# claymore666/openhush

Measured on AMD Instinct MI355X. Metric: audio-sec/sec (xRT) large-v3 greedy, 30s chunks, 1/2/4/8 MI355X, higher is better.
Workload: dtype bf16; 1 GPU; large-v3 dims, steps of batch=32 x 30 s windows per GPU, greedy, 100 tokens/window (EOT suppressed), procedural weights seed 1234, every window a distinct synthetic recording, PCM resident in HBM; schedule LANES 4x3: 12 steps (384 windows) in flight per GPU - per lane ONE front-end pass and ONE decode batch of 96 rows, 4 decodes side by side on 64 CUs each; concurrent_sub_batches=1

## Files before the change

### include/ohw.h

```cpp
#ifndef OHW_H
#define OHW_H

#include <stddef.h>
#include <stdint.h>

#ifdef __cplusplus
extern "C" {
#endif

#define OHW_ABI_VERSION 2

enum {
  OHW_OK = 0,
  OHW_E_MODEL_NOT_FOUND = -3001,
  OHW_E_LOAD_FAILED = -3002,
  OHW_E_TRANSCRIBE = -3003,
  OHW_E_NO_GPU = -3004,
  OHW_E_OOM = -3005,
  OHW_E_INVALID_ARG = -3006,
  OHW_E_VALIDATION = -3007
};

enum { OHW_DTYPE_AUTO = -1, OHW_DTYPE_BF16 = 0, OHW_DTYPE_F16 = 1 };

// ... 464 lines not shown
int ohw_pool_set_fallback_device(ohw_pool* p, int on);
int ohw_pool_set_window_mode(ohw_pool* p, int mode);
int ohw_pool_set_initial_prompt(ohw_pool* p, const char* text);
int ohw_pool_set_hot_phrases(ohw_pool* p, const char* const* texts, const float* boosts, int n);
int ohw_pool_set_repetition(ohw_pool* p, float penalty, int ngram);
int ohw_pool_set_commands(ohw_pool* p, const char* const* texts, int n, float penalty);
int ohw_pool_set_best_of(ohw_pool* p, int n);
int ohw_pool_set_carry_context(ohw_pool* p, int max_tokens);
int ohw_pool_set_audio_ctx(ohw_pool* p, int n);
int ohw_pool_set_packed_encoder(ohw_pool* p, int on);
int ohw_pool_set_detect_language(ohw_pool* p, int on);
const char* ohw_pool_broadcast_note(const ohw_pool* p);
int ohw_pool_n_devices(const ohw_pool* p);
const char* ohw_pool_broadcast_kind(const ohw_pool* p);
ohw_engine* ohw_pool_engine(ohw_pool* p, int i);
void ohw_pool_free(ohw_pool* p);

const char* ohw_lang_id_to_code(int32_t id);
int32_t ohw_lang_code_to_id(const char* code);

const char* ohw_last_error(void);
int ohw_abi_version(void);
int ohw_state_fetch(ohw_state* st, const char* what, int batch, float* out, int64_t out_elems);
int ohw_ctx_weight_digest(const ohw_ctx* ctx, int index, char* name_out , uint64_t* digest);
int ohw_dequantize_host(int ttype, const void* blocks, int64_t n, float* out);
int ohw_dbg_dequantize(int device, int ttype, const void* blocks_host, int64_t n, float* out_host);
int ohw_dbg_gemm(int dtype, const void* A, const void* W, const float* bias, void* out, int64_t M, int64_t N,
                 int64_t K, int epilogue, void* stream);
int ohw_dbg_gemm_small(int dtype, const void* A, const void* W, const float* bias, void* out, int64_t M, int64_t N,
                       int64_t K, int epilogue, void* stream);
int ohw_dbg_attention(int dtype, const void* qkv, void* out, int batch, int T, int n_head, void* stream);
int ohw_dbg_attention_var(int dtype, const void* qkv, void* out, int batch, int T, int n_head, const int32_t* win_len_host,
                          const int32_t* win_off_host, void* stream);
enum { OHW_XA_PLAIN = 0, OHW_XA_SPLIT, OHW_XA_ROWS2, OHW_XA_ROWS3, OHW_XA_ROWS4, OHW_XA_GROUP2, OHW_XA_GROUP3, OHW_XA_GROUP4,
       OHW_XA_GROUP5, OHW_XA_GROUP_SPLIT };
enum { OHW_SA_PLAIN = 0, OHW_SA_SLOTS };
int ohw_dbg_cross_attn(int dtype, const void* q, const void* xk, const void* xv, void* out, int M, int n_new, int n_head, int t_len,
                       int kv_group, int batch_invariant, const int32_t* done_host, const int32_t* win_len_host, float* partials,
                       unsigned* tickets, int max_split_rows, int* variant_out, void* stream);
int ohw_dbg_cross_attn_chunk(int dtype, const void* q, const void* xk, const void* xv, void* out, int windows, int n_head, int t_len,
                             const int32_t* win_len_host, const int32_t* done_host, void* stream);
int ohw_dbg_cross_attn_chunk_n(int dtype, const void* q, const void* xk, const void* xv, void* out, int windows, int n_head, int t_len,
                               const int32_t* win_len_host, const int32_t* done_host, void* stream, int n_q);
int ohw_dbg_self_attn(int dtype, const void* q, const void* k_cache, const void* v_cache, const int32_t* n_past_host, void* out, int M,
                      int n_new, int n_head, int n_ctx, const int32_t* kv_slot_host, int* variant_out, void* stream);
int ohw_dbg_align_probs(int dtype, const void* q, const void* xk, int rows, int n_head, int t_len, int n_keys,
                        const int32_t* heads_host, int n_heads, float* p_out_host, void* stream);
int ohw_dbg_align_reduce(int device, const float* p_host, int n_heads, int n_all, int n_prompt, int n_keys, float* m_out_host);
int ohw_dbg_dtw(int device, const float* m_host, int n, int n_keys, int32_t* start_idx_out);
int ohw_dbg_poison(ohw_state* st, const char* what);
int ohw_dbg_vad_energy(ohw_state* st, const float* pcm, int64_t n, int pcm_on_device, float* e_out, int guard);
int ohw_dbg_vad_floor(ohw_state* st, const float* e, int64_t n_frames, const ohw_vad_detector* d, float* prob_out, int guard, float* floor_db_out);
int ohw_dbg_sample(ohw_state* st, const ohw_sample_params* p, const float* logits, const int32_t* history, int hist_stride,
                   const int32_t* n_hist, int batch, int32_t* tokens_out, float* logprobs_out, float* no_speech_out);
int ohw_dbg_sample_t(ohw_state* st, const ohw_sample_params* p, const float* logits, const int32_t* history, int hist_stride,
                     const int32_t* n_hist, int batch, float temperature, const double* uniforms, int32_t* tokens_out,
                     float* logprobs_out, float* no_speech_out);
int ohw_dbg_sample_group(ohw_state* st, const ohw_sample_params* p, const float* logits, const int32_t* history, int hist_stride,
                         const int32_t* n_hist, int n_windows, int group, int first, float temperature, const double* uniforms,
                         int32_t* done, int32_t* tokens_out, float* logprobs_out, float* no_speech_out, int32_t* win_done_out,
                         int32_t* n_cur_out);
int ohw_dbg_lang_pick(ohw_state* st, const float* logits, int batch, int32_t* ids_out, float* probs_out);
int ohw_dbg_counter(const ohw_state* st, const char* name);

#define OHW_DBG_SENTINEL_I32 (-7777777)
#define OHW_DBG_SENTINEL_F32 (-12345.0f)
// ... 133 lines not shown
```

### openhush_amd/csrc/attention.hip

```cpp
#include <type_traits>

#include "attention.hpp"

namespace ohw {

constexpr int ATT_THREADS = 256;
constexpr int ATT_QROWS = 128;
constexpr int ATT_KB = 64;

__device__ __forceinline__ int k_swz(int row) { return (row >> 1) & 7; }
__device__ __forceinline__ int v_swz(int row) { return ((row >> 1) & 1) << 2; }

enum AttMode { ATT_UNIFORM = 0, ATT_VAR = 1, ATT_PACKED = 2 };

template <typename T, int MODE>
__device__ __forceinline__ void encoder_attention_body(const T* __restrict__ qkv, T* __restrict__ out, int batch, int t_len, int n_head,
                                                       const int32_t* __restrict__ win_len, const int32_t* __restrict__ win_off) {
  using Ops = TypeOps<T>;
  using vec8 = typename Ops::vec8;
  __shared__ __attribute__((aligned(16))) unsigned char smem[2 * 16384];
  const int tid = threadIdx.x, lane = tid & 63, wave = tid >> 6;
  const int d = n_head * 64;
  const int64_t ld = 3 * (int64_t)d;
  const int nqb = (t_len + ATT_QROWS - 1) / ATT_QROWS;
  const unsigned nwg = (unsigned)(nqb * n_head * batch);
  const unsigned lid = xcd_remap(blockIdx.x, nwg);
  const int qb = lid % nqb;
  const int bh = lid / nqb;
  const int h = bh % n_head, b = bh / n_head;

  const int t_stride = t_len;
  int64_t row0 = (int64_t)b * t_stride;
  if (MODE == ATT_PACKED) {
    t_len = win_len[b];
    if (qb * ATT_QROWS >= t_len) return;
    row0 = win_off[b];
  }
  if (MODE == ATT_VAR) {
    t_len = win_len[b];
    if (qb * ATT_QROWS >= t_len) {
      const int r = qb * ATT_QROWS + (tid >> 1);
      if (r < t_stride) {
        u32x4* o = (u32x4*)(out + ((int64_t)b * t_stride + r) * d + h * 64 + (tid & 1) * 32);
        const u32x4 z = {0u, 0u, 0u, 0u};
#pragma unroll
        for (int i = 0; i < 4; ++i) o[i] = z;
      }
      return;
// ... 11 lines not shown

  const int skey = tid >> 3, schunk = tid & 7;
  const T* kg = base + d + h * 64 + schunk * 8;
  const T* vg = base + 2 * d + h * 64 + schunk * 8;
  int k_lds[2], v_lds[2];
#pragma unroll
  for (int i = 0; i < 2; ++i) {
    const int r = skey + 32 * i;
    k_lds[i] = r * 128 + ((schunk ^ k_swz(r)) << 4);
    v_lds[i] = 8192 + r * 128 + ((schunk ^ v_swz(r)) << 4);
  }
  const int nkb = (t_len + ATT_KB - 1) / ATT_KB;
  u32x4 rk[2][2], rv[2][2];
  auto gload = [&](auto set, int kb) {
    constexpr int S = decltype(set)::value;
#pragma unroll
    for (int i = 0; i < 2; ++i) {
      int key = kb * ATT_KB + skey + 32 * i;
      if (key > t_len - 1) key = t_len - 1;
      rk[S][i] = *(const u32x4*)(kg + (int64_t)key * ld);
      rv[S][i] = *(const u32x4*)(vg + (int64_t)key * ld);
    }
  };
  auto lstore = [&](auto set, int stage) {
    constexpr int S = decltype(set)::value;
#pragma unroll
    for (int i = 0; i < 2; ++i) {
      *(u32x4*)(smem + stage * 16384 + k_lds[i]) = rk[S][i];
      *(u32x4*)(smem + stage * 16384 + v_lds[i]) = rv[S][i];
    }
  };
  using Set0 = std::integral_constant<int, 0>;
  using Set1 = std::integral_constant<int, 1>;
  gload(Set0{}, 0);
  lstore(Set0{}, 0);
  __syncthreads();

  int k_rd[2];
#pragma unroll
  for (int kt = 0; kt < 2; ++kt) k_rd[kt] = (kt * 32 + ql) * 128;
  const int ksw = k_swz(ql);
  const int tq = (lane & 15) >> 2, tp = lane & 3, tg = (lane >> 4) & 1;

  f32x16 oacc[2];
#pragma unroll
  for (int i = 0; i < 2; ++i)
#pragma unroll
    for (int r = 0; r < 16; ++r) oacc[i][r] = 0.f;
  float m_run = -INFINITY, l_run = 0.f;
  const float sc = 0.125f * 1.44269504088896340736f;

  if (nkb > 1) gload(Set1{}, 1);
  auto block = [&](auto set, int kb) {
    constexpr int S = decltype(set)::value;
    const int cur = S * 16384;
    const bool more = kb + 1 < nkb;
    if (kb + 2 < nkb) gload(std::integral_constant<int, S>{}, kb + 2);

    f32x16 sacc[2];
#pragma unroll
    for (int kt = 0; kt < 2; ++kt) {
#pragma unroll
      for (int r = 0; r < 16; ++r) sacc[kt][r] = 0.f;
#pragma unroll
      for (int ks = 0; ks < 4; ++ks) {
        vec8 kf = *(const vec8*)(smem + cur + k_rd[kt] + (((2 * ks + hh) ^ ksw) << 4));
        sacc[kt] = Ops::mfma32(kf, qf[ks], sacc[kt]);
      }
    }
    const int key0 = kb * ATT_KB;
    if (key0 + ATT_KB > t_len) {
#pragma unroll
      for (int kt = 0; kt < 2; ++kt)
#pragma unroll
        for (int r = 0; r < 16; ++r) {
          const int key = key0 + kt * 32 + (r & 3) + 8 * (r >> 2) + 4 * hh;
          sacc[kt][r] = key < t_len ? sacc[kt][r] : -INFINITY;
        }
    }
    float bmax = -INFINITY;
#pragma unroll
    for (int kt = 0; kt < 2; ++kt)
#pragma unroll
      for (int r = 0; r < 16; ++r) bmax = fmaxf(bmax, sacc[kt][r]);
    bmax = fmaxf(bmax, __shfl_xor(bmax, 32, 64));
    const float m_new = fmaxf(m_run, bmax);
    if (!__all(m_new == m_run)) {
      const float alpha = __builtin_amdgcn_exp2f((m_run - m_new) * sc);
      l_run *= alpha;
#pragma unroll
// ... 4 lines not shown
    }
    const float m_sc = m_run * sc;
    float psum = 0.f;
#pragma unroll
    for (int kt = 0; kt < 2; ++kt)
#pragma unroll
      for (int r = 0; r < 16; ++r) {
        const float pv = __builtin_amdgcn_exp2f(__builtin_fmaf(sacc[kt][r], sc, -m_sc));
        sacc[kt][r] = pv;
        psum += pv;
      }
    l_run += psum;

#pragma unroll
    for (int sp = 0; sp < 4; ++sp) {
      const int kt = sp >> 1, s = sp & 1;
      union { vec8 v; unsigned u[4]; } pf;
#pragma unroll
      for (int j = 0; j < 4; ++j) pf.u[j] = pack2<T>(sacc[kt][8 * s + 2 * j], sacc[kt][8 * s + 2 * j + 1]);
      const int kbase = kt * 32 + 16 * s + 4 * hh + tq;
#pragma unroll
      for (int dt = 0; dt < 2; ++dt) {
        union { vec8 v; s16x4 h4[2]; } vf;
#pragma unroll
        for (int jj = 0; jj < 2; ++jj) {
          const int row = kbase + 8 * jj;
          const int colb = (dt * 32 + 16 * tg + 4 * tp) * 2;
          const int off = cur + 8192 + row * 128 + ((((colb >> 4) ^ v_swz(row)) << 4) | (colb & 15));
          vf.h4[jj] = __builtin_amdgcn_ds_read_tr16_b64_v4i16((__attribute__((address_space(3))) s16x4*)(smem + off));
        }
        oacc[dt] = Ops::mfma32(vf.v, pf.v, oacc[dt]);
      }
    }
    if (more) lstore(std::integral_constant<int, 1 - S>{}, 1 - S);
    __syncthreads();
  };
  for (int kb = 0; kb < nkb; kb += 2) {
    block(Set0{}, kb);
    if (kb + 1 < nkb) block(Set1{}, kb + 1);
  }

  l_run += __shfl_xor(l_run, 32, 64);
  const float inv = 1.0f / l_run;
  if (q_valid) {
    T* o = out + (row0 + q_row) * d + h * 64;
#pragma unroll
    for (int dt = 0; dt < 2; ++dt)
#pragma unroll
      for (int g = 0; g < 4; ++g) {
        u32x2 w;
        w.x = pack2<T>(oacc[dt][4 * g] * inv, oacc[dt][4 * g + 1] * inv);
        w.y = pack2<T>(oacc[dt][4 * g + 2] * inv, oacc[dt][4 * g + 3] * inv);
        *(u32x2*)(o + dt * 32 + 8 * g + 4 * hh) = w;
      }
  }
}

template <typename T, bool VAR>
__global__ __launch_bounds__(ATT_THREADS, 2) void encoder_attention_kernel(const T* __restrict__ qkv, T* __restrict__ out,
                                                                          int batch, int t_len, int n_head, const int32_t* __restrict__ win_len) {
  encoder_attention_body<T, VAR ? ATT_VAR : ATT_UNIFORM>(qkv, out, batch, t_len, n_head, win_len, nullptr);
}
template <typename T>
__global__ __launch_bounds__(ATT_THREADS, 2) void encoder_attention_packed_kernel(const T* __restrict__ qkv, T* __restrict__ out, int batch, int t_len, int n_head,
                                                                                 const int32_t* __restrict__ win_len, const int32_t* __restrict__ win_off) {
  encoder_attention_body<T, ATT_PACKED>(qkv, out, batch, t_len, n_head, win_len, win_off);
}

template <typename T>
void launch_encoder_attention(const void* qkv, void* out, int batch, int t_len, int n_head, hipStream_t stream, const int32_t* win_len, const int32_t* win_off) {
  const int nqb = (t_len + ATT_QROWS - 1) / ATT_QROWS;
  const unsigned nwg = (unsigned)(nqb * n_head * batch);
  if (win_off && !win_len) throw Error(OHW_E_INVALID_ARG, "attention: packed rows need the windows' lengths");
  if (win_off)
    hipLaunchKernelGGL((encoder_attention_packed_kernel<T>), dim3(nwg), dim3(ATT_THREADS), 0, stream, (const T*)qkv, (T*)out, batch, t_len, n_head, win_len, win_off);
  else if (win_len)
    hipLaunchKernelGGL((encoder_attention_kernel<T, true>), dim3(nwg), dim3(ATT_THREADS), 0, stream, (const T*)qkv, (T*)out, batch, t_len, n_head, win_len);
  else
    hipLaunchKernelGGL((encoder_attention_kernel<T, false>), dim3(nwg), dim3(ATT_THREADS), 0, stream, (const T*)qkv, (T*)out, batch, t_len, n_head, win_len);
  HIP_CHECK(hipGetLastError());
}
template void launch_encoder_attention<bf16_t>(const void*, void*, int, int, int, hipStream_t, const int32_t*, const int32_t*);
template void launch_encoder_attention<f16_t>(const void*, void*, int, int, int, hipStream_t, const int32_t*, const int32_t*);

}
```

### openhush_amd/csrc/attention.hpp

```cpp
#pragma once
#include "common.hpp"

namespace ohw {
template <typename T> void launch_encoder_attention(const void* qkv, void* out, int batch, int t_len, int n_head, hipStream_t stream,
                                                    const int32_t* win_len = nullptr, const int32_t* win_off = nullptr);
}
```

### openhush_amd/csrc/engine.hip

```cpp
#include <execinfo.h>
#include <signal.h>
#include <unistd.h>

#include <cstring>
#include <memory>
#include <mutex>
#include <shared_mutex>
#include <type_traits>
#include <vector>
#include <algorithm>

#include "attention.hpp"
#include "dequant.hpp"
#include "gemm.hpp"
#include "kernels.hpp"
#include "logit_rules.hpp"
#include "model.hpp"

namespace ohw {
ohw_ctx* ctx_from_file(const char* path, int device, int dtype);
ohw_ctx* ctx_synthetic(const ohw_hparams* hp, uint32_t seed, int device, int dtype);
ohw_ctx* ctx_shell(const ohw_hparams* hp, int device, int dtype);
void select_device(int device);

// ... 3152 lines not shown
    HIP_CHECK(hipStreamSynchronize(nullptr));
    HIP_CHECK(hipMemcpy(out_host, out.p, (size_t)n * 4, hipMemcpyDeviceToHost));
  });
}

int ohw_dbg_poison(ohw_state* st, const char* what) {
  return guard([&] {
    if (!st || !what) throw Error(OHW_E_INVALID_ARG, "null argument");
    const std::string w = what;
    const DevBuf* buf = w == "qkv" ? &st->qkv : w == "att" ? &st->att : nullptr;
    if (!buf) throw Error(OHW_E_INVALID_ARG, std::string("poison: unknown buffer '") + what + "'");
    HIP_CHECK(hipSetDevice(st->ctx->device));
    HIP_CHECK(hipMemsetAsync(buf->p, 0xff, buf->bytes, st->stream));
  });
}

int ohw_dbg_attention(int dtype, const void* qkv, void* out, int batch, int T, int n_head, void* stream) {
  return guard([&] {
    Dispatch::run(dtype, [&](auto* tag) {
      using TT = std::remove_pointer_t<decltype(tag)>;
      launch_encoder_attention<TT>(qkv, out, batch, T, n_head, (hipStream_t)stream);
    });
  });
}

static void dbg_upload(DevBuf& buf, const int32_t* host, size_t n) {
  buf.alloc(n * sizeof(int32_t));
  HIP_CHECK(hipMemcpy(buf.p, host, n * sizeof(int32_t), hipMemcpyHostToDevice));
}
static void dbg_check_dtype(int dtype, const char* what) {
  if (dtype != OHW_DTYPE_BF16 && dtype != OHW_DTYPE_F16) throw Error(OHW_E_INVALID_ARG, std::string(what) + ": dtype must be 0 (bf16) or 1 (f16)");
}

int ohw_dbg_attention_var(int dtype, const void* qkv, void* out, int batch, int T, int n_head, const int32_t* win_len_host,
                          const int32_t* win_off_host, void* stream) {
  return guard([&] {
    dbg_check_dtype(dtype, "dbg_attention_var");
    if (!qkv || !out || batch < 1 || T < 1 || n_head < 1) throw Error(OHW_E_INVALID_ARG, "dbg_attention_var: null buffer, or batch, T or n_head below 1");
    if (win_off_host && !win_len_host) throw Error(OHW_E_INVALID_ARG, "dbg_attention_var: packed rows (win_off) need the windows' lengths (win_len)");
    int64_t sum = 0;
    for (int b = 0; win_len_host && b < batch; ++b) {
      if (win_len_host[b] < 1 || win_len_host[b] > T)
        throw Error(OHW_E_INVALID_ARG, "dbg_attention_var: win_len[" + std::to_string(b) + "] = " + std::to_string(win_len_host[b]) + " is outside 1 .. T = " + std::to_string(T));
      if (win_off_host && win_off_host[b] != sum)
        throw Error(OHW_E_INVALID_ARG, "dbg_attention_var: win_off[" + std::to_string(b) + "] = " + std::to_string(win_off_host[b]) +
                                           " is not the exclusive prefix sum of win_len (" + std::to_string(sum) + ")");
      sum += win_len_host[b];
    }
    DevBuf len, off;
    if (win_len_host) dbg_upload(len, win_len_host, (size_t)batch);
    if (win_off_host) dbg_upload(off, win_off_host, (size_t)batch);
    Dispatch::run(dtype, [&](auto* tag) {
      using TT = std::remove_pointer_t<decltype(tag)>;
      launch_encoder_attention<TT>(qkv, out, batch, T, n_head, (hipStream_t)stream, win_len_host ? len.as<int32_t>() : nullptr,
                                   win_off_host ? off.as<int32_t>() : nullptr);
    });
    HIP_CHECK(hipStreamSynchronize((hipStream_t)stream));
  });
}

int ohw_dbg_cross_attn(int dtype, const void* q, const void* xk, const void* xv, void* out, int M, int n_new, int n_head, int t_len,
                       int kv_group, int batch_invariant, const int32_t* done_host, const int32_t* win_len_host, float* partials,
                       unsigned* tickets, int max_split_rows, int* variant_out, void* stream) {
  return guard([&] {
    dbg_check_dtype(dtype, "dbg_cross_attn");
    if (!q || !xk || !xv || !out || M < 1 || n_new < 1 || n_head < 1 || t_len < 1)
      throw Error(OHW_E_INVALID_ARG, "dbg_cross_attn: null buffer, or M, n_new, n_head or t_len below 1");
    if (kv_group < 1 || kv_group > 5) throw Error(OHW_E_INVALID_ARG, "dbg_cross_attn: kv_group must be 1 .. 5 (beams per window)");
    if (kv_group > 1 && n_new != 1) throw Error(OHW_E_INVALID_ARG, "dbg_cross_attn: beams (kv_group > 1) are single-token rows: n_new must be 1");
    if (M % n_new != 0) throw Error(OHW_E_INVALID_ARG, "dbg_cross_attn: M must be a multiple of n_new");
    if (kv_group > 1 && M % kv_group != 0) throw Error(OHW_E_INVALID_ARG, "dbg_cross_attn: M must be a multiple of kv_group");
    if ((partials == nullptr) != (tickets == nullptr)) throw Error(OHW_E_INVALID_ARG, "dbg_cross_attn: partials and tickets come together");
    if (partials && !batch_invariant && !win_len_host && (max_split_rows < 1 || M > max_split_rows))
      throw Error(OHW_E_INVALID_ARG, "dbg_cross_attn: M = " + std::to_string(M) + " rows exceed max_split_rows = " + std::to_string(max_split_rows) +
                                         ", the rows the partials and tickets hold");
    const int windows = kv_group > 1 ? M / kv_group : M / n_new;
    for (int w = 0; win_len_host && w < windows; ++w)
      if (win_len_host[w] < 1 || win_len_host[w] > t_len)
        throw Error(OHW_E_INVALID_ARG, "dbg_cross_attn: win_len[" + std::to_string(w) + "] = " + std::to_string(win_len_host[w]) + " is outside 1 .. t_len = " + std::to_string(t_len));
    DevBuf done, len;
    if (done_host) dbg_upload(done, done_host, (size_t)windows);
    if (win_len_host) dbg_upload(len, win_len_host, (size_t)windows);
    int variant = -1;
    Dispatch::run(dtype, [&](auto* tag) {
      using TT = std::remove_pointer_t<decltype(tag)>;
      variant = launch_cross_attn<TT>(q, xk, xv, out, M, n_new, n_head, t_len, partials, tickets, max_split_rows,
                                      done_host ? done.as<int32_t>() : nullptr, (hipStream_t)stream, kv_group, batch_invariant != 0,
                                      win_len_host ? len.as<int32_t>() : nullptr);
    });
    HIP_CHECK(hipStreamSynchronize((hipStream_t)stream));
// ... 337 lines not shown
```

### openhush_amd/engine.py

```python
from __future__ import annotations

import ctypes as C
import dataclasses
import os
import time
from typing import List, Optional, Sequence, Tuple, Union

import numpy as np

_HERE = os.path.dirname(os.path.abspath(__file__))
LIB_PATH = os.environ.get("OHW_LIB") or os.path.join(_HERE, "libohw.so")

CHUNK_SAMPLES = 480000
CHUNK_FRAMES = 3000

OHW_DTYPE_AUTO, OHW_DTYPE_BF16, OHW_DTYPE_F16 = -1, 0, 1
OHW_MEL_REFLECT, OHW_MEL_ZERO_TAIL = 0, 1
OHW_WINDOW_FIXED, OHW_WINDOW_SEEK, OHW_WINDOW_FIXED_RECORDING_MEL = 0, 1, 2
OHW_SCHEDULE_SEQUENTIAL, OHW_SCHEDULE_PIPELINE, OHW_SCHEDULE_LANES = 0, 1, 2
EPI_BIAS_T, EPI_BIAS_GELU_T, EPI_BIAS_RESID_F32, EPI_F32 = 0, 1, 2, 4
XA_PLAIN, XA_SPLIT, XA_ROWS2, XA_ROWS3, XA_ROWS4, XA_GROUP2, XA_GROUP3, XA_GROUP4, XA_GROUP5, XA_GROUP_SPLIT = range(10)
SA_PLAIN, SA_SLOTS = 0, 1

OHW_E_MODEL_NOT_FOUND, OHW_E_LOAD_FAILED, OHW_E_TRANSCRIBE = -3001, -3002, -3003
OHW_E_NO_GPU, OHW_E_OOM, OHW_E_INVALID_ARG, OHW_E_VALIDATION = -3004, -3005, -3006, -3007


class HParams(C.Structure):
    _fields_ = [(n, C.c_int32) for n in ("n_vocab", "n_audio_ctx", "n_audio_state", "n_audio_head", "n_audio_layer",
                                         "n_text_ctx", "n_text_state", "n_text_head", "n_text_layer", "n_mels", "ftype")]

    def as_list(self):
        return [int(getattr(self, n)) for n, _ in self._fields_]


class SpecialTokens(C.Structure):
    _fields_ = [(n, C.c_int32) for n in ("eot", "sot", "translate", "transcribe", "solm", "prev", "nosp", "no_timestamps",
                                         "timestamp_begin", "blank", "n_langs")]


class AudioInfo(C.Structure):
    _fields_ = [("error", C.c_int32), ("duration_secs", C.c_float), ("sample_count", C.c_int64), ("min_value", C.c_float),
                ("max_value", C.c_float), ("rms", C.c_float), ("nan_count", C.c_int64), ("inf_count", C.c_int64)]


class SampleParams(C.Structure):
    _fields_ = [(n, C.c_int32) for n in ("lang_id", "translate", "no_timestamps", "suppress_blank", "max_initial_ts", "n_max", "force_len")]


class PreprocessConfig(C.Structure):
    _fields_ = [("preprocessing", C.c_int32), ("normalization_enabled", C.c_int32), ("normalization_target_db", C.c_float),
                ("compression_enabled", C.c_int32), ("compression_threshold_db", C.c_float), ("compression_ratio", C.c_float),
                ("compression_attack_ms", C.c_float), ("compression_release_ms", C.c_float), ("compression_makeup_gain_db", C.c_float),
                ("limiter_enabled", C.c_int32), ("limiter_ceiling_db", C.c_float), ("limiter_release_ms", C.c_float)]

# ... 431 lines not shown


AUDIO_ERRORS = {0: "Ok", 1: "Empty", 2: "InvalidSampleRate", 3: "TooLong", 4: "TooShort", 5: "ContainsNaN", 6: "ContainsInfinite"}

EXPORTS = [
    "ohw_validate_audio", "ohw_ctx_create", "ohw_ctx_create_synthetic", "ohw_ctx_info", "ohw_token_text", "ohw_ctx_free",
    "ohw_state_create", "ohw_state_free", "ohw_state_set_stream", "ohw_state_max_batch", "ohw_mel", "ohw_recording_set", "ohw_mel_seek", "ohw_encode", "ohw_decode",
    "ohw_default_sample_params", "ohw_sample_greedy_host", "ohw_greedy", "ohw_state_timings", "ohw_engine_new",
    "ohw_engine_transcribe", "ohw_engine_last_tokens", "ohw_engine_benchmark", "ohw_engine_free", "ohw_engine_state",
    "ohw_engine_ctx", "ohw_lang_id_to_code", "ohw_lang_code_to_id", "ohw_last_error", "ohw_abi_version", "ohw_state_fetch",
    "ohw_dbg_gemm", "ohw_dbg_attention", "ohw_state_profile_begin", "ohw_state_profile_end", "ohw_ctx_weight_digest", "ohw_detect_language", "ohw_state_ctx", "ohw_engine_set_window_mode", "ohw_engine_last_text", "ohw_engine_last_quality",
    "ohw_stream_create", "ohw_stream_destroy", "ohw_stream_wait", "ohw_stream_sync",
    "ohw_ctx_create_shell", "ohw_ctx_blob_size", "ohw_ctx_blob_export", "ohw_ctx_blob_import",
    "ohw_default_preprocess_config", "ohw_preprocess_audio", "ohw_dsp_rms_db", "ohw_dsp_apply_gain", "ohw_dsp_normalize_rms",
    "ohw_dsp_compress", "ohw_dsp_limit", "ohw_dsp_resample_linear",
    "ohw_tracker_new", "ohw_tracker_free", "ohw_tracker_add_pending", "ohw_tracker_add_result", "ohw_tracker_take_ready", "ohw_tracker_ready_get",
    "ohw_tracker_reset_dedup", "ohw_tracker_is_empty", "ohw_tracker_is_pending", "ohw_tracker_pending_count", "ohw_tracker_waiting_count", "ohw_extract_chunk",
    "ohw_chunk_scheduler_new", "ohw_chunk_scheduler_free", "ohw_chunk_scheduler_tick", "ohw_chunk_scheduler_position", "ohw_chunk_scheduler_next_id",
    "ohw_chunk_scheduler_rejected", "ohw_resampler_create", "ohw_resampler_free", "ohw_resampler_out_len", "ohw_resampler_run", "ohw_greedy_ex", "ohw_state_set_logit_bias", "ohw_state_set_batch_invariant", "ohw_dbg_sample",
    "ohw_decode_active", "ohw_rng_new", "ohw_rng_free", "ohw_sample_host", "ohw_default_decode_policy", "ohw_engine_set_decode_policy",
    "ohw_engine_last_trace", "ohw_engine_set_schedule", "ohw_ctx_dtype",
    "ohw_beam_search", "ohw_encode_slice", "ohw_dsp_resample_sinc", "ohw_default_vad_config", "ohw_vad_state_new", "ohw_vad_state_free", "ohw_vad_state_update",
    "ohw_vad_state_is_speech", "ohw_vad_state_speech_start", "ohw_vad_state_reset", "ohw_vad_energy_engine", "ohw_vad_energy_engine_free",
    "ohw_vad_run",
    "ohw_pool_create", "ohw_pool_transcribe", "ohw_pool_last_text", "ohw_pool_last_tokens", "ohw_pool_last_quality",
    "ohw_dbg_counter", "ohw_dsp_denoise", "ohw_denoise_passthrough_engine", "ohw_preprocess_audio_ex", "ohw_pool_set_window_mode",
    "ohw_state_set_persistent", "ohw_pool_broadcast_note", "ohw_pool_create_synthetic", "ohw_pool_set_force_len", "ohw_pool_set_schedule", "ohw_engine_set_force_len",
    "ohw_pool_set_decode_policy", "ohw_pool_n_devices", "ohw_pool_broadcast_kind", "ohw_pool_engine", "ohw_pool_free",
    "ohw_rng_uniforms", "ohw_rng_discard_draws", "ohw_sample_pass", "ohw_dbg_sample_t", "ohw_engine_set_fallback_device",
    "ohw_pool_set_fallback_device", "ohw_dequantize_host", "ohw_dbg_dequantize",
    "ohw_state_set_audio_ctx", "ohw_state_audio_ctx", "ohw_audio_ctx_for", "ohw_engine_set_audio_ctx", "ohw_pool_set_audio_ctx", "ohw_dbg_gemm_small",
    "ohw_state_set_window_ctx", "ohw_state_window_ctx", "ohw_engine_transcribe_batch", "ohw_engine_batch_result", "ohw_batch_plan",
    "ohw_state_set_packed_encoder", "ohw_state_packed_encoder", "ohw_engine_set_packed_encoder", "ohw_pool_set_packed_encoder", "ohw_dbg_poison",
    "ohw_dbg_attention_var", "ohw_dbg_cross_attn", "ohw_dbg_self_attn",
    "ohw_engine_set_detect_language", "ohw_engine_last_language", "ohw_engine_transcribe_batch_lang", "ohw_pool_set_detect_language",
    "ohw_state_set_window_lang", "ohw_state_detect_window_lang", "ohw_state_window_lang", "ohw_lang_pick_host", "ohw_dbg_lang_pick",
    "ohw_state_set_align_heads", "ohw_state_align", "ohw_align_reduce_host", "ohw_dtw_host", "ohw_dbg_align_probs", "ohw_dbg_align_reduce",
    "ohw_dbg_dtw", "ohw_engine_set_word_timestamps", "ohw_engine_last_token_times", "ohw_engine_last_words", "ohw_engine_last_segments",
    "ohw_engine_batch_times", "ohw_word_starts_host", "ohw_segments_host",
    "ohw_pool_set_word_timestamps", "ohw_pool_last_token_times", "ohw_pool_last_words", "ohw_pool_last_segments",
    "ohw_dbg_beam_step", "ohw_beam_search_ex", "ohw_dbg_beam_step_ex", "ohw_dbg_beam_finish", "ohw_beam_finish_host",
    "ohw_engine_set_beam_size", "ohw_pool_set_beam_size",
    "ohw_dbg_cross_attn_chunk",
    "ohw_state_set_window_prompt", "ohw_state_window_prompt_len", "ohw_state_prefill", "ohw_tokenize_host", "ohw_tokenize", "ohw_prompt_clip_host",
    "ohw_engine_set_initial_prompt", "ohw_engine_set_initial_prompt_tokens", "ohw_pool_set_initial_prompt",
    "ohw_recording_set_slot", "ohw_mel_seek_slots", "ohw_seek_sched_new", "ohw_seek_sched_round", "ohw_seek_sched_advance", "ohw_seek_sched_free",
    "ohw_engine_transcribe_long_batch", "ohw_engine_long_batch_quality",
    "ohw_dbg_dec_gemm", "ohw_dbg_embed", "ohw_dbg_layernorm",
    "ohw_state_set_prefill_chunk", "ohw_state_prefill_chunk", "ohw_engine_set_prefill_chunk", "ohw_dbg_cross_attn_chunk_n",
    "ohw_engine_set_carry_context", "ohw_pool_set_carry_context", "ohw_engine_last_context", "ohw_engine_long_batch_context", "ohw_carry_step_host",
    "ohw_seq_eval_host", "ohw_needs_fallback_host",
    "ohw_sample_pass_n", "ohw_dbg_sample_group", "ohw_best_of_pick_host", "ohw_engine_set_best_of", "ohw_pool_set_best_of",
    "ohw_engine_last_candidates", "ohw_engine_last_candidate_logprobs", "ohw_batch_windows_host",
    "ohw_dbg_enc_gemm",
    "ohw_phrase_table_build_host", "ohw_phrase_boost_host", "ohw_state_set_phrase_table", "ohw_state_phrase_count", "ohw_dbg_phrase_boost",
    "ohw_engine_set_hot_phrases", "ohw_engine_set_hot_phrases_tokens", "ohw_pool_set_hot_phrases",
    "ohw_repeat_rule_host", "ohw_state_set_repeat_rule", "ohw_state_repeat_rule", "ohw_dbg_repeat_rule", "ohw_engine_set_repetition",
    "ohw_pool_set_repetition",
    "ohw_command_table_build_host", "ohw_command_rule_host", "ohw_command_match_host", "ohw_state_set_command_table", "ohw_state_command_count",
    "ohw_state_command_list_logprob", "ohw_dbg_command_rule", "ohw_engine_set_commands", "ohw_engine_set_commands_tokens", "ohw_pool_set_commands",
    "ohw_engine_last_commands", "ohw_engine_batch_commands",
    "ohw_dbg_sample_ex",
    "ohw_default_vad_detector", "ohw_state_vad_frames", "ohw_speech_segments_host", "ohw_default_chunk_plan", "ohw_speech_chunks_host",
    "ohw_engine_set_vad", "ohw_engine_transcribe_speech", "ohw_engine_transcribe_speech_lang", "ohw_engine_speech_chunks",
    "ohw_engine_speech_segments", "ohw_dbg_vad_energy", "ohw_dbg_vad_floor",
    "ohw_state_score", "ohw_state_set_score_buffers", "ohw_token_score_host", "ohw_token_prob_host", "ohw_word_probs_host",
    "ohw_dbg_token_score", "ohw_dbg_logits_rows",
# ... 213 lines not shown
        L.ohw_engine_set_window_mode.argtypes = [vp, C.c_int]
        L.ohw_engine_set_schedule.argtypes = [vp, C.c_int, C.c_int, C.c_int]
        L.ohw_engine_last_quality.argtypes = [vp, C.POINTER(C.POINTER(WindowQuality)), C.POINTER(C.c_int)]
        L.ohw_engine_last_text.argtypes = [vp, C.POINTER(C.c_char_p), C.POINTER(C.c_size_t)]
        L.ohw_engine_last_tokens.argtypes = [vp, C.POINTER(ip), C.POINTER(C.c_int)]
        L.ohw_engine_benchmark.argtypes = [vp, C.c_float, fp, fp, fp]
        L.ohw_engine_free.argtypes = [vp]
        L.ohw_engine_free.restype = None
        L.ohw_engine_state.argtypes = [vp]
        L.ohw_engine_state.restype = vp
        L.ohw_engine_ctx.argtypes = [vp]
        L.ohw_engine_ctx.restype = vp
        L.ohw_pool_create.argtypes = [C.c_char_p, C.c_char_p, C.c_int, ip, C.c_int, C.c_int, C.c_int, C.POINTER(vp)]
        L.ohw_pool_transcribe.argtypes = [vp, fp, C.c_int64, C.c_uint32, C.c_char_p, C.c_size_t, C.c_char_p, C.POINTER(C.c_uint64), C.POINTER(AudioInfo)]
        L.ohw_pool_last_text.argtypes = [vp, C.POINTER(C.c_char_p), C.POINTER(C.c_size_t)]
        L.ohw_pool_last_tokens.argtypes = [vp, C.POINTER(ip), C.POINTER(C.c_int)]
        L.ohw_pool_last_quality.argtypes = [vp, C.POINTER(C.POINTER(WindowQuality)), C.POINTER(C.c_int)]
        L.ohw_pool_set_decode_policy.argtypes = [vp, C.POINTER(DecodePolicy)]
        L.ohw_pool_n_devices.argtypes = [vp]
        L.ohw_pool_broadcast_kind.argtypes = [vp]
        L.ohw_pool_broadcast_kind.restype = C.c_char_p
        L.ohw_pool_engine.argtypes = [vp, C.c_int]
        L.ohw_pool_engine.restype = vp
        L.ohw_pool_free.argtypes = [vp]
        L.ohw_pool_free.restype = None
        L.ohw_state_fetch.argtypes = [vp, C.c_char_p, C.c_int, fp, C.c_int64]
        L.ohw_state_profile_begin.argtypes = [vp, C.c_int]
        L.ohw_state_profile_end.argtypes = [vp, C.POINTER(C.c_int64), C.POINTER(C.c_double), C.POINTER(C.c_double)]
        L.ohw_ctx_weight_digest.argtypes = [vp, C.c_int, C.c_char_p, C.POINTER(C.c_uint64)]
        L.ohw_dbg_gemm.argtypes = [C.c_int, vp, vp, vp, vp, C.c_int64, C.c_int64, C.c_int64, C.c_int, vp]
        L.ohw_dbg_attention.argtypes = [C.c_int, vp, vp, C.c_int, C.c_int, C.c_int, vp]
        L.ohw_dbg_gemm_small.argtypes = [C.c_int, vp, vp, vp, vp, C.c_int64, C.c_int64, C.c_int64, C.c_int, vp]
        L.ohw_dbg_attention_var.argtypes = [C.c_int, vp, vp, C.c_int, C.c_int, C.c_int, ip, ip, vp]
        L.ohw_dbg_cross_attn.argtypes = [C.c_int, vp, vp, vp, vp, C.c_int, C.c_int, C.c_int, C.c_int, C.c_int, C.c_int, ip, ip, vp, vp, C.c_int,
                                         C.POINTER(C.c_int), vp]
        L.ohw_dbg_cross_attn_chunk.argtypes = [C.c_int, vp, vp, vp, vp, C.c_int, C.c_int, C.c_int, ip, ip, vp]
        L.ohw_state_set_window_prompt.argtypes = [vp, ip, C.c_int, ip, C.c_int]
        L.ohw_state_window_prompt_len.argtypes = [vp, C.c_int]
        L.ohw_state_prefill.argtypes = [vp, C.c_int, ip]
        L.ohw_tokenize_host.argtypes = [C.c_char_p, ip, C.c_int, C.c_char_p, ip, C.c_int]
        L.ohw_tokenize.argtypes = [vp, C.c_char_p, ip, C.c_int]
        L.ohw_prompt_clip_host.argtypes = [ip, C.c_int, C.c_int, ip]
        L.ohw_engine_set_initial_prompt.argtypes = [vp, C.c_char_p]
        L.ohw_engine_set_initial_prompt_tokens.argtypes = [vp, ip, C.c_int]
        L.ohw_pool_set_initial_prompt.argtypes = [vp, C.c_char_p]
        L.ohw_engine_set_carry_context.argtypes = [vp, C.c_int]
        L.ohw_state_set_prefill_chunk.argtypes = [vp, C.c_int]
        L.ohw_state_prefill_chunk.argtypes = [vp]
        L.ohw_engine_set_prefill_chunk.argtypes = [vp, C.c_int]
        L.ohw_dbg_cross_attn_chunk_n.argtypes = [C.c_int, vp, vp, vp, vp, C.c_int, C.c_int, C.c_int, ip, ip, vp, C.c_int]
        L.ohw_pool_set_carry_context.argtypes = [vp, C.c_int]
        L.ohw_engine_last_context.argtypes = [vp, C.c_int, C.POINTER(C.POINTER(C.c_int32)), C.POINTER(C.c_int)]
        L.ohw_engine_long_batch_context.argtypes = [vp, C.c_int, C.c_int, C.POINTER(C.POINTER(C.c_int32)), C.POINTER(C.c_int)]
        L.ohw_carry_step_host.argtypes = [ip, C.POINTER(C.c_int), C.c_int, ip, C.c_int, C.c_float, C.c_int, ip, C.POINTER(C.c_int)]
        L.ohw_dbg_self_attn.argtypes = [C.c_int, vp, vp, vp, ip, vp, C.c_int, C.c_int, C.c_int, C.c_int, ip, C.POINTER(C.c_int), vp]
        L.ohw_dbg_dec_gemm.argtypes = [C.POINTER(DbgDecGemmIO), vp]
        L.ohw_dbg_enc_gemm.argtypes = [C.POINTER(DbgEncGemmIO), vp]
        L.ohw_dbg_embed.argtypes = [C.c_int, vp, C.c_int, vp, C.c_int, ip, ip, vp, vp, vp, C.c_int, C.c_int, C.c_int, vp]
        L.ohw_dbg_layernorm.argtypes = [C.c_int, vp, vp, vp, vp, C.c_int64, C.c_int, C.c_int, vp]
        L.ohw_dbg_logits_rows.argtypes = [C.POINTER(DbgLogitsRowsIO), vp]
        L.ohw_state_score.argtypes = [vp, C.POINTER(SampleParams), ip, C.c_int, ip, C.c_int, vp, ip, ip]
        L.ohw_state_set_score_buffers.argtypes = [vp, C.c_int]
        L.ohw_token_score_host.argtypes = [fp, C.c_int, C.c_int, C.c_int, C.POINTER(TokenScore)]
        L.ohw_token_prob_host.argtypes = [C.POINTER(TokenScore), fp, fp, fp]
        L.ohw_word_probs_host.argtypes = [fp, ip, C.c_int, fp]
        L.ohw_dbg_token_score.argtypes = [vp, fp, C.c_int, C.c_int64, C.c_int, C.c_int, ip, ip, C.c_int, C.c_int, C.c_int, C.c_int, vp]
# ... 2149 lines not shown
```

Measured before the change: 4095 audio-sec/sec.

## Stage encoder attention K/V through global-to-LDS DMA instead of registers

```diff
diff --git a/include/ohw.h b/include/ohw.h
--- a/include/ohw.h
+++ b/include/ohw.h
@@ -520,6 +520,9 @@
 int ohw_dbg_attention(int dtype, const void* qkv, void* out, int batch, int T, int n_head, void* stream);
 int ohw_dbg_attention_var(int dtype, const void* qkv, void* out, int batch, int T, int n_head, const int32_t* win_len_host,
                           const int32_t* win_off_host, void* stream);
+enum { OHW_ATT_FORM_REGS = 0, OHW_ATT_FORM_DMA = 1 };
+int ohw_dbg_attention_form(int dtype, const void* qkv, void* out, int batch, int T, int n_head, const int32_t* win_len_host,
+                           const int32_t* win_off_host, int form, int* form_out, void* stream);
 enum { OHW_XA_PLAIN = 0, OHW_XA_SPLIT, OHW_XA_ROWS2, OHW_XA_ROWS3, OHW_XA_ROWS4, OHW_XA_GROUP2, OHW_XA_GROUP3, OHW_XA_GROUP4,
        OHW_XA_GROUP5, OHW_XA_GROUP_SPLIT };
 enum { OHW_SA_PLAIN = 0, OHW_SA_SLOTS };
diff --git a/openhush_amd/csrc/attention.hip b/openhush_amd/csrc/attention.hip
--- a/openhush_amd/csrc/attention.hip
+++ b/openhush_amd/csrc/attention.hip
@@ -1,3 +1,5 @@
+#include <cstdlib>
+#include <string>
 #include <type_traits>
 
 #include "attention.hpp"
@@ -12,8 +14,9 @@
 __device__ __forceinline__ int v_swz(int row) { return ((row >> 1) & 1) << 2; }
 
 enum AttMode { ATT_UNIFORM = 0, ATT_VAR = 1, ATT_PACKED = 2 };
-
-template <typename T, int MODE>
+enum AttForm { ATT_REGS = OHW_ATT_FORM_REGS, ATT_DMA = OHW_ATT_FORM_DMA };
+
+template <typename T, int MODE, int FORM>
 __device__ __forceinline__ void encoder_attention_body(const T* __restrict__ qkv, T* __restrict__ out, int batch, int t_len, int n_head,
                                                        const int32_t* __restrict__ win_len, const int32_t* __restrict__ win_off) {
   using Ops = TypeOps<T>;
@@ -91,9 +94,42 @@
   };
   using Set0 = std::integral_constant<int, 0>;
   using Set1 = std::integral_constant<int, 1>;
-  gload(Set0{}, 0);
-  lstore(Set0{}, 0);
-  __syncthreads();
+
+  const int wave_u = __builtin_amdgcn_readfirstlane(wave);
+  const T* kd = base + d + h * 64 + (schunk ^ k_swz(skey)) * 8;
+  const T* vd = base + 2 * d + h * 64 + (schunk ^ v_swz(skey)) * 8;
+  auto dma = [&](int kb, int stage) {
+#pragma unroll
+    for (int i = 0; i < 2; ++i) {
+      int key = kb * ATT_KB + skey + 32 * i;
+      if (key > t_len - 1) key = t_len - 1;
+      unsigned char* piece = smem + stage * 16384 + (wave_u * 8 + 32 * i) * 128;
+      __builtin_amdgcn_global_load_lds((const __attribute__((address_space(1))) void*)(kd + (int64_t)key * ld),
+                                       (__attribute__((address_space(3))) void*)piece, 16, 0, 0);
+      __builtin_amdgcn_global_load_lds((const __attribute__((address_space(1))) void*)(vd + (int64_t)key * ld),
+                                       (__attribute__((address_space(3))) void*)(piece + 8192), 16, 0, 0);
+    }
+  };
+  auto ring_wait = [&]() {
+    asm volatile("s_waitcnt vmcnt(0) lgkmcnt(0)" ::: "memory");
+    __builtin_amdgcn_s_barrier();
+    __builtin_amdgcn_sched_barrier(0);
+  };
+  if constexpr (FORM == ATT_DMA) {
+    dma(0, 0);
+    if (nkb > 1) {
+      dma(1, 1);
+      asm volatile("s_waitcnt vmcnt(4)" ::: "memory");
+    } else {
+      asm volatile("s_waitcnt vmcnt(0)" ::: "memory");
+    }
+    __builtin_amdgcn_s_barrier();
+    __builtin_amdgcn_sched_barrier(0);
+  } else {
+    gload(Set0{}, 0);
+    lstore(Set0{}, 0);
+    __syncthreads();
+  }
 
   int k_rd[2];
 #pragma unroll
@@ -109,12 +145,16 @@
   float m_run = -INFINITY, l_run = 0.f;
   const float sc = 0.125f * 1.44269504088896340736f;
 
-  if (nkb > 1) gload(Set1{}, 1);
+  if constexpr (FORM == ATT_REGS) {
+    if (nkb > 1) gload(Set1{}, 1);
+  }
   auto block = [&](auto set, int kb) {
     constexpr int S = decltype(set)::value;
     const int cur = S * 16384;
     const bool more = kb + 1 < nkb;
-    if (kb + 2 < nkb) gload(std::integral_constant<int, S>{}, kb + 2);
+    if constexpr (FORM == ATT_REGS) {
+      if (kb + 2 < nkb) gload(std::integral_constant<int, S>{}, kb + 2);
+    }
 
     f32x16 sacc[2];
 #pragma unroll
@@ -185,8 +225,13 @@
         oacc[dt] = Ops::mfma32(vf.v, pf.v, oacc[dt]);
       }
     }
-    if (more) lstore(std::integral_constant<int, 1 - S>{}, 1 - S);
-    __syncthreads();
+    if constexpr (FORM == ATT_DMA) {
+      ring_wait();
+      if (kb + 2 < nkb) dma(kb + 2, S);
+    } else {
+      if (more) lstore(std::integral_constant<int, 1 - S>{}, 1 - S);
+      __syncthreads();
+    }
   };
   for (int kb = 0; kb < nkb; kb += 2) {
     block(Set0{}, kb);
@@ -209,31 +254,41 @@
   }
 }
 
-template <typename T, bool VAR>
-__global__ __launch_bounds__(ATT_THREADS, 2) void encoder_attention_kernel(const T* __restrict__ qkv, T* __restrict__ out,
+template <typename T, bool VAR, int FORM>
+__global__ __launch_bounds__(ATT_THREADS, FORM == ATT_DMA ? 4 : 2) void encoder_attention_kernel(const T* __restrict__ qkv, T* __restrict__ out,
                                                                           int batch, int t_len, int n_head, const int32_t* __restrict__ win_len) {
-  encoder_attention_body<T, VAR ? ATT_VAR : ATT_UNIFORM>(qkv, out, batch, t_len, n_head, win_len, nullptr);
-}
+  encoder_attention_body<T, VAR ? ATT_VAR : ATT_UNIFORM, FORM>(qkv, out, batch, t_len, n_head, win_len, nullptr);
+}
+template <typename T, int FORM>
+__global__ __launch_bounds__(ATT_THREADS, FORM == ATT_DMA ? 4 : 2) void encoder_attention_packed_kernel(const T* __restrict__ qkv, T* __restrict__ out, int batch, int t_len, int n_head,
+                                                                                 const int32_t* __restrict__ win_len, const int32_t* __restrict__ win_off) {
+  encoder_attention_body<T, ATT_PACKED, FORM>(qkv, out, batch, t_len, n_head, win_len, win_off);
+}
+
+template <typename T, int FORM>
+static void launch_form(const T* qkv, T* out, int batch, int t_len, int n_head, hipStream_t stream, const int32_t* win_len, const int32_t* win_off, unsigned nwg) {
+  if (win_off)
+    hipLaunchKernelGGL((encoder_attention_packed_kernel<T, FORM>), dim3(nwg), dim3(ATT_THREADS), 0, stream, qkv, out, batch, t_len, n_head, win_len, win_off);
+  else if (win_len)
+    hipLaunchKernelGGL((encoder_attention_kernel<T, true, FORM>), dim3(nwg), dim3(ATT_THREADS), 0, stream, qkv, out, batch, t_len, n_head, win_len);
+  else
+    hipLaunchKernelGGL((encoder_attention_kernel<T, false, FORM>), dim3(nwg), dim3(ATT_THREADS), 0, stream, qkv, out, batch, t_len, n_head, win_len);
+}
+
 template <typename T>
-__global__ __launch_bounds__(ATT_THREADS, 2) void encoder_attention_packed_kernel(const T* __restrict__ qkv, T* __restrict__ out, int batch, int t_len, int n_head,
-                                                                                 const int32_t* __restrict__ win_len, const int32_t* __restrict__ win_off) {
-  encoder_attention_body<T, ATT_PACKED>(qkv, out, batch, t_len, n_head, win_len, win_off);
-}
-
-template <typename T>
-void launch_encoder_attention(const void* qkv, void* out, int batch, int t_len, int n_head, hipStream_t stream, const int32_t* win_len, const int32_t* win_off) {
+int launch_encoder_attention(const void* qkv, void* out, int batch, int t_len, int n_head, hipStream_t stream, const int32_t* win_len, const int32_t* win_off, int form) {
   const int nqb = (t_len + ATT_QROWS - 1) / ATT_QROWS;
   const unsigned nwg = (unsigned)(nqb * n_head * batch);
   if (win_off && !win_len) throw Error(OHW_E_INVALID_ARG, "attention: packed rows need the windows' lengths");
-  if (win_off)
-    hipLaunchKernelGGL((encoder_attention_packed_kernel<T>), dim3(nwg), dim3(ATT_THREADS), 0, stream, (const T*)qkv, (T*)out, batch, t_len, n_head, win_len, win_off);
-  else if (win_len)
-    hipLaunchKernelGGL((encoder_attention_kernel<T, true>), dim3(nwg), dim3(ATT_THREADS), 0, stream, (const T*)qkv, (T*)out, batch, t_len, n_head, win_len);
-  else
-    hipLaunchKernelGGL((encoder_attention_kernel<T, false>), dim3(nwg), dim3(ATT_THREADS), 0, stream, (const T*)qkv, (T*)out, batch, t_len, n_head, win_len);
+  if (form < -1 || form > ATT_DMA) throw Error(OHW_E_INVALID_ARG, "attention: form must be -1 (the configured one), 0 (registers) or 1 (LDS-DMA)");
+  static const int form_env = [] { const char* e = getenv("OHW_ATT_STAGE"); return e && std::string(e) == "regs" ? (int)ATT_REGS : (int)ATT_DMA; }();
+  if (form < 0) form = form_env;
+  if (form == ATT_DMA) launch_form<T, ATT_DMA>((const T*)qkv, (T*)out, batch, t_len, n_head, stream, win_len, win_off, nwg);
+  else launch_form<T, ATT_REGS>((const T*)qkv, (T*)out, batch, t_len, n_head, stream, win_len, win_off, nwg);
   HIP_CHECK(hipGetLastError());
-}
-template void launch_encoder_attention<bf16_t>(const void*, void*, int, int, int, hipStream_t, const int32_t*, const int32_t*);
-template void launch_encoder_attention<f16_t>(const void*, void*, int, int, int, hipStream_t, const int32_t*, const int32_t*);
-
-}
+  return form;
+}
+template int launch_encoder_attention<bf16_t>(const void*, void*, int, int, int, hipStream_t, const int32_t*, const int32_t*, int);
+template int launch_encoder_attention<f16_t>(const void*, void*, int, int, int, hipStream_t, const int32_t*, const int32_t*, int);
+
+}
diff --git a/openhush_amd/csrc/attention.hpp b/openhush_amd/csrc/attention.hpp
--- a/openhush_amd/csrc/attention.hpp
+++ b/openhush_amd/csrc/attention.hpp
@@ -2,6 +2,6 @@
 #include "common.hpp"
 
 namespace ohw {
-template <typename T> void launch_encoder_attention(const void* qkv, void* out, int batch, int t_len, int n_head, hipStream_t stream,
-                                                    const int32_t* win_len = nullptr, const int32_t* win_off = nullptr);
+template <typename T> int launch_encoder_attention(const void* qkv, void* out, int batch, int t_len, int n_head, hipStream_t stream,
+                                                   const int32_t* win_len = nullptr, const int32_t* win_off = nullptr, int form = -1);
 }
diff --git a/openhush_amd/csrc/engine.hip b/openhush_amd/csrc/engine.hip
--- a/openhush_amd/csrc/engine.hip
+++ b/openhush_amd/csrc/engine.hip
@@ -3208,9 +3208,10 @@
   if (dtype != OHW_DTYPE_BF16 && dtype != OHW_DTYPE_F16) throw Error(OHW_E_INVALID_ARG, std::string(what) + ": dtype must be 0 (bf16) or 1 (f16)");
 }
 
-int ohw_dbg_attention_var(int dtype, const void* qkv, void* out, int batch, int T, int n_head, const int32_t* win_len_host,
-                          const int32_t* win_off_host, void* stream) {
-  return guard([&] {
+static int dbg_attention_run(int dtype, const void* qkv, void* out, int batch, int T, int n_head, const int32_t* win_len_host,
+                             const int32_t* win_off_host, int form, void* stream) {
+  int ran = -1;
+  {
     dbg_check_dtype(dtype, "dbg_attention_var");
     if (!qkv || !out || batch < 1 || T < 1 || n_head < 1) throw Error(OHW_E_INVALID_ARG, "dbg_attention_var: null buffer, or batch, T or n_head below 1");
     if (win_off_host && !win_len_host) throw Error(OHW_E_INVALID_ARG, "dbg_attention_var: packed rows (win_off) need the windows' lengths (win_len)");
@@ -3228,10 +3229,26 @@
     if (win_off_host) dbg_upload(off, win_off_host, (size_t)batch);
     Dispatch::run(dtype, [&](auto* tag) {
       using TT = std::remove_pointer_t<decltype(tag)>;
-      launch_encoder_attention<TT>(qkv, out, batch, T, n_head, (hipStream_t)stream, win_len_host ? len.as<int32_t>() : nullptr,
-                                   win_off_host ? off.as<int32_t>() : nullptr);
+      ran = launch_encoder_attention<TT>(qkv, out, batch, T, n_head, (hipStream_t)stream, win_len_host ? len.as<int32_t>() : nullptr,
+                                         win_off_host ? off.as<int32_t>() : nullptr, form);
     });
     HIP_CHECK(hipStreamSynchronize((hipStream_t)stream));
+  }
+  return ran;
+}
+
+int ohw_dbg_attention_var(int dtype, const void* qkv, void* out, int batch, int T, int n_head, const int32_t* win_len_host,
+                          const int32_t* win_off_host, void* stream) {
+  return guard([&] { dbg_attention_run(dtype, qkv, out, batch, T, n_head, win_len_host, win_off_host, -1, stream); });
+}
+
+int ohw_dbg_attention_form(int dtype, const void* qkv, void* out, int batch, int T, int n_head, const int32_t* win_len_host,
+                           const int32_t* win_off_host, int form, int* form_out, void* stream) {
+  return guard([&] {
+    if (form != -1 && form != OHW_ATT_FORM_REGS && form != OHW_ATT_FORM_DMA)
+      throw Error(OHW_E_INVALID_ARG, "dbg_attention_form: form must be -1 (the configured one), 0 (registers) or 1 (LDS-DMA)");
+    const int ran = dbg_attention_run(dtype, qkv, out, batch, T, n_head, win_len_host, win_off_host, form, stream);
+    if (form_out) *form_out = ran;
   });
 }
 
diff --git a/openhush_amd/engine.py b/openhush_amd/engine.py
--- a/openhush_amd/engine.py
+++ b/openhush_amd/engine.py
@@ -21,6 +21,7 @@
 EPI_BIAS_T, EPI_BIAS_GELU_T, EPI_BIAS_RESID_F32, EPI_F32 = 0, 1, 2, 4
 XA_PLAIN, XA_SPLIT, XA_ROWS2, XA_ROWS3, XA_ROWS4, XA_GROUP2, XA_GROUP3, XA_GROUP4, XA_GROUP5, XA_GROUP_SPLIT = range(10)
 SA_PLAIN, SA_SLOTS = 0, 1
+ATT_FORM_REGS, ATT_FORM_DMA = 0, 1
 
 OHW_E_MODEL_NOT_FOUND, OHW_E_LOAD_FAILED, OHW_E_TRANSCRIBE = -3001, -3002, -3003
 OHW_E_NO_GPU, OHW_E_OOM, OHW_E_INVALID_ARG, OHW_E_VALIDATION = -3004, -3005, -3006, -3007
@@ -518,7 +519,7 @@
     "ohw_state_set_audio_ctx", "ohw_state_audio_ctx", "ohw_audio_ctx_for", "ohw_engine_set_audio_ctx", "ohw_pool_set_audio_ctx", "ohw_dbg_gemm_small",
     "ohw_state_set_window_ctx", "ohw_state_window_ctx", "ohw_engine_transcribe_batch", "ohw_engine_batch_result", "ohw_batch_plan",
     "ohw_state_set_packed_encoder", "ohw_state_packed_encoder", "ohw_engine_set_packed_encoder", "ohw_pool_set_packed_encoder", "ohw_dbg_poison",
-    "ohw_dbg_attention_var", "ohw_dbg_cross_attn", "ohw_dbg_self_attn",
+    "ohw_dbg_attention_var", "ohw_dbg_attention_form", "ohw_dbg_cross_attn", "ohw_dbg_self_attn",
     "ohw_engine_set_detect_language", "ohw_engine_last_language", "ohw_engine_transcribe_batch_lang", "ohw_pool_set_detect_language",
     "ohw_state_set_window_lang", "ohw_state_detect_window_lang", "ohw_state_window_lang", "ohw_lang_pick_host", "ohw_dbg_lang_pick",
     "ohw_state_set_align_heads", "ohw_state_align", "ohw_align_reduce_host", "ohw_dtw_host", "ohw_dbg_align_probs", "ohw_dbg_align_reduce",
@@ -798,6 +799,7 @@
         L.ohw_dbg_attention.argtypes = [C.c_int, vp, vp, C.c_int, C.c_int, C.c_int, vp]
         L.ohw_dbg_gemm_small.argtypes = [C.c_int, vp, vp, vp, vp, C.c_int64, C.c_int64, C.c_int64, C.c_int, vp]
         L.ohw_dbg_attention_var.argtypes = [C.c_int, vp, vp, C.c_int, C.c_int, C.c_int, ip, ip, vp]
+        L.ohw_dbg_attention_form.argtypes = [C.c_int, vp, vp, C.c_int, C.c_int, C.c_int, ip, ip, C.c_int, C.POINTER(C.c_int), vp]
         L.ohw_dbg_cross_attn.argtypes = [C.c_int, vp, vp, vp, vp, C.c_int, C.c_int, C.c_int, C.c_int, C.c_int, C.c_int, ip, ip, vp, vp, C.c_int,
                                          C.POINTER(C.c_int), vp]
         L.ohw_dbg_cross_attn_chunk.argtypes = [C.c_int, vp, vp, vp, vp, C.c_int, C.c_int, C.c_int, ip, ip, vp]
```

Result: no change. 4094 audio-sec/sec (median of 2 runs) (-0.0%).
